# facebookresearch/dpr-scale

Hardware: NVIDIA H100
Metric: query+ctx pairs/sec (BERT-base, seq128) (higher is better)
Workload: dtype bf16

## Files before the change

dpr_scale_b200/csrc/attention.cu:

```cuda
#include "attention.cuh"
#include "dprb_internal.h"

namespace dprb {
namespace {

constexpr int DH = 64;
constexpr int SHORT_MAX = 256;

int check_shape(int nseq, int S, int heads, const char* who) {
  DPRB_REQUIRE(nseq >= 0 && heads > 0, "%s: bad nseq=%d heads=%d", who, nseq, heads);
  DPRB_REQUIRE(S >= 1 && S <= 512, "%s: sequence length %d unsupported (1..512)", who, S);
  return 0;
}

}

int attn_fwd_lse(const void* qkv, const int32_t* attn_mask, void* ctx, float* lse, int nseq, int S, int heads,
                 float dropout_p, unsigned long long site_seed, cudaStream_t stream) {
  if (int rc = check_shape(nseq, S, heads, "attn_fwd")) return rc;
  if (nseq == 0) return 0;
  if (S > SHORT_MAX) return attn_fwd_long(qkv, attn_mask, ctx, lse, nseq, S, heads, dropout_p, site_seed, stream);
  return attn_fwd_wg(qkv, attn_mask, ctx, lse, nseq, S, heads, dropout_p, site_seed, stream);
}

int attn_bwd_lse(const void* qkv, const int32_t* attn_mask, const void* ctx, const float* lse, const void* dctx,
                 void* dqkv, float* dbias, int nseq, int S, int heads, float dropout_p,
                 unsigned long long site_seed, cudaStream_t stream) {
  if (int rc = check_shape(nseq, S, heads, "attn_bwd")) return rc;
  if (nseq == 0) return 0;
  if (S > SHORT_MAX) {
    if (int rc = attn_bwd_long(qkv, attn_mask, ctx, lse, dctx, dqkv, nseq, S, heads, dropout_p, site_seed, stream)) return rc;
  } else {
    if (int rc = attn_bwd_wg(qkv, attn_mask, lse, dctx, dqkv, nseq, S, heads, dropout_p, site_seed, stream)) return rc;
  }
  if (dbias != nullptr) return colsum_bf16(dqkv, 3LL * heads * DH, dbias, nseq * S, 3 * heads * DH, stream);
  return 0;
}

}
```

dpr_scale_b200/csrc/attention_wgmma.cu:

```cuda
#include "attention.cuh"
#include "dprb_internal.h"

namespace dprb {
namespace {

template <int N>
__device__ __forceinline__ void mma_ss(float (&d)[N / 2], uint64_t a, uint64_t b, int acc) {
  if constexpr (N == 64) wgmma_m64n64_ss_bf16<0, 0>(d, a, b, acc);
  else if constexpr (N == 128) wgmma_m64n128_ss_bf16<0, 0>(d, a, b, acc);
  else wgmma_m64n256_ss_bf16<0, 0>(d, a, b, acc);
}

template <int NK>
constexpr int fwd_smem() { return 64 * 128 + 2 * NK * 128 + NK * 4 + 16 + 1024; }

template <int NK, bool DROP>
__global__ void __launch_bounds__(128)
attn_fwd_wg_kernel(const __grid_constant__ CUtensorMap tm_q, const __grid_constant__ CUtensorMap tm_kv,
                   const int32_t* __restrict__ attn_mask, bf16* __restrict__ ctx, float* __restrict__ lse_out, int S,
                   int heads, Drop drop) {
  extern __shared__ uint8_t smem_raw[];
  uint8_t* smem = align1024(smem_raw);
  uint8_t* sQ = smem;
  uint8_t* sK = sQ + 64 * 128;
  uint8_t* sV = sK + NK * 128;
  float* sMask = reinterpret_cast<float*>(sV + NK * 128);
  uint64_t* bar = reinterpret_cast<uint64_t*>(sMask + NK);

  const int tid = threadIdx.x, warp = tid >> 5, lane = tid & 31, q4 = lane & 3;
  const int nqb = (S + 63) / 64;
  const int prob = blockIdx.x / nqb, qb = blockIdx.x - prob * nqb;
  const int seq = prob / heads, h = prob - seq * heads;
  const int H = heads * 64;
  if (tid == 0) {
    tma_prefetch_desc(&tm_q);
    tma_prefetch_desc(&tm_kv);
    mbar_init(bar, 1);
    fence_barrier_init();
  }
  __syncthreads();
  if (tid == 0) {
    mbar_arrive_expect_tx(bar, 64 * 128 + 2 * NK * 128);
    tma_load_3d(sQ, &tm_q, bar, h * 64, qb * 64, seq);
    tma_load_3d(sK, &tm_kv, bar, H + h * 64, 0, seq);
    tma_load_3d(sV, &tm_kv, bar, 2 * H + h * 64, 0, seq);
  }
  for (int j = tid; j < NK; j += 128) {
    const bool keep = j < S && (attn_mask == nullptr || attn_mask[(long long)seq * S + j] != 0);
    sMask[j] = keep ? 0.f : -INFINITY;
  }
  __syncthreads();
  mbar_wait(bar, 0);

  float s[NK / 2];
  wgmma_fence();
#pragma unroll
  for (int k = 0; k < 4; ++k) mma_ss<NK>(s, desc_k(sQ) + k * KSTEP_K, desc_k(sK) + k * KSTEP_K, k > 0);
  wgmma_commit();
  wgmma_wait<0>();

  const int lrow = warp * 16 + (lane >> 2);
  float m[2] = {-INFINITY, -INFINITY};
#pragma unroll
  for (int c = 0; c < NK / 8; ++c) {
    const float2 mk = *reinterpret_cast<const float2*>(sMask + 8 * c + 2 * q4);
#pragma unroll
    for (int h2 = 0; h2 < 2; ++h2) {
      float& x = s[4 * c + 2 * h2];
      float& y = s[4 * c + 2 * h2 + 1];
      x = fmaf(x, ATTN_SCALE_LOG2, mk.x);
      y = fmaf(y, ATTN_SCALE_LOG2, mk.y);
      m[h2] = fmaxf(m[h2], fmaxf(x, y));
    }
  }
  float l[2] = {0.f, 0.f};
#pragma unroll
  for (int h2 = 0; h2 < 2; ++h2) {
    m[h2] = fmaxf(m[h2], __shfl_xor_sync(0xFFFFFFFFu, m[h2], 1));
    m[h2] = fmaxf(m[h2], __shfl_xor_sync(0xFFFFFFFFu, m[h2], 2));
  }
  const float e[2] = {m[0] == -INFINITY ? 0.f : m[0], m[1] == -INFINITY ? 0.f : m[1]};
  uint32_t pk[NK / 4];
#pragma unroll
  for (int c = 0; c < NK / 8; ++c) {
#pragma unroll
    for (int h2 = 0; h2 < 2; ++h2) {
      float px = ex2_approx(s[4 * c + 2 * h2] - e[h2]);
      float py = ex2_approx(s[4 * c + 2 * h2 + 1] - e[h2]);
      l[h2] += px + py;
      if (DROP) {
        float m0, m1;
        drop.mul2((uint32_t)(prob * S + qb * 64 + lrow + 8 * h2), (uint32_t)(8 * c + 2 * q4), m0, m1);
        px *= m0; py *= m1;
      }
      pk[2 * c + h2] = pack_bf16x2(px, py);
    }
  }
#pragma unroll
  for (int h2 = 0; h2 < 2; ++h2) {
    l[h2] += __shfl_xor_sync(0xFFFFFFFFu, l[h2], 1);
    l[h2] += __shfl_xor_sync(0xFFFFFFFFu, l[h2], 2);
  }

  float o[32];
  wgmma_fence();
#pragma unroll
  for (int j = 0; j < NK / 16; ++j) {
    const uint32_t a[4] = {pk[4 * j], pk[4 * j + 1], pk[4 * j + 2], pk[4 * j + 3]};
    wgmma_m64n64_rs_bf16<1>(o, a, desc_mn(sV) + j * KSTEP_MN, j > 0);
  }
  wgmma_commit();
  wgmma_wait<0>();

#pragma unroll
  for (int h2 = 0; h2 < 2; ++h2) {
    const int row = qb * 64 + lrow + 8 * h2;
    if (row >= S) continue;
    if (lse_out != nullptr && q4 == 0) lse_out[(long long)prob * S + row] = m[h2] * ATTN_LN2 + __logf(l[h2]);
    const float inv = l[h2] > 0.f ? 1.f / l[h2] : 0.f;
    bf16* dst = ctx + ((long long)seq * S + row) * H + h * 64;
#pragma unroll
    for (int c = 0; c < 8; ++c)
      *reinterpret_cast<uint32_t*>(dst + 8 * c + 2 * q4) = pack_bf16x2(o[4 * c + 2 * h2] * inv, o[4 * c + 2 * h2 + 1] * inv);
  }
}

template <int NK>
constexpr int bwd_smem() { return 4 * NK * 128 + NK * 256 + 2 * 8192 + 3 * NK * 4 + 16 + 1024; }

template <int NK, bool DROP>
__global__ void __launch_bounds__(256, 1)
attn_bwd_wg_kernel(const __grid_constant__ CUtensorMap tm_qkv, const __grid_constant__ CUtensorMap tm_do,
                   const int32_t* __restrict__ attn_mask, const float* __restrict__ lse_in, bf16* __restrict__ dqkv, int S,
                   int heads, Drop drop) {
  extern __shared__ uint8_t smem_raw[];
  uint8_t* smem = align1024(smem_raw);
  uint8_t* sQ = smem;
  uint8_t* sdO = sQ + NK * 128;
  uint8_t* sK = sdO + NK * 128;
  uint8_t* sV = sK + NK * 128;
  float* sdQ = reinterpret_cast<float*>(sV + NK * 128);
  uint8_t* sStage = reinterpret_cast<uint8_t*>(sdQ + NK * 64);
  float* sLse = reinterpret_cast<float*>(sStage + 2 * 8192);
  float* sD = sLse + NK;
  float* sMask = sD + NK;
  uint64_t* bar = reinterpret_cast<uint64_t*>(sMask + NK);

  const int tid = threadIdx.x, warp = tid >> 5, lane = tid & 31, q4 = lane & 3;
  const int wg = warp >> 2;
  const int prob = blockIdx.x, seq = prob / heads, h = prob - seq * heads;
  const int H = heads * 64;
  if (tid == 0) {
    tma_prefetch_desc(&tm_qkv);
    tma_prefetch_desc(&tm_do);
    mbar_init(bar, 1);
    fence_barrier_init();
  }
  __syncthreads();
  if (tid == 0) {
    mbar_arrive_expect_tx(bar, 4 * NK * 128);
    tma_load_3d(sQ, &tm_qkv, bar, h * 64, 0, seq);
    tma_load_3d(sdO, &tm_do, bar, h * 64, 0, seq);
    tma_load_3d(sK, &tm_qkv, bar, H + h * 64, 0, seq);
    tma_load_3d(sV, &tm_qkv, bar, 2 * H + h * 64, 0, seq);
  }
  for (int i = tid; i < NK * 64; i += 256) sdQ[i] = 0.f;
  for (int j = tid; j < NK; j += 256) {
    const bool keep = j < S && (attn_mask == nullptr || attn_mask[(long long)seq * S + j] != 0);
    sMask[j] = keep ? 0.f : -INFINITY;
    sLse[j] = j < S ? lse_in[(long long)prob * S + j] * ATTN_LOG2E : INFINITY;
    sD[j] = 0.f;
  }
  __syncthreads();
  mbar_wait(bar, 0);

  const int nblk = (S + 63) / 64;
  const int lrow = (warp & 3) * 16 + (lane >> 2);
  for (int qb = wg; qb < nblk; qb += 2) {
    float Dr[2] = {0.f, 0.f};
    const float ls[2] = {sLse[qb * 64 + lrow], sLse[qb * 64 + lrow + 8]};
    for (int kc = 0; kc < nblk; ++kc) {
      float sc[32], dp[32];
      wgmma_fence();
#pragma unroll
      for (int k = 0; k < 4; ++k) wgmma_m64n64_ss_bf16<0, 0>(sc, desc_k(sQ + qb * 8192) + k * KSTEP_K, desc_k(sK + kc * 8192) + k * KSTEP_K, k > 0);
#pragma unroll
      for (int k = 0; k < 4; ++k) wgmma_m64n64_ss_bf16<0, 0>(dp, desc_k(sdO + qb * 8192) + k * KSTEP_K, desc_k(sV + kc * 8192) + k * KSTEP_K, k > 0);
      wgmma_commit();
      wgmma_wait<0>();
#pragma unroll
      for (int c = 0; c < 8; ++c) {
        const int kcol = kc * 64 + 8 * c + 2 * q4;
        const float2 mk = *reinterpret_cast<const float2*>(sMask + kcol);
#pragma unroll
        for (int h2 = 0; h2 < 2; ++h2) {
          const int i = 4 * c + 2 * h2;
          float px = ex2_approx(fmaf(sc[i], ATTN_SCALE_LOG2, mk.x) - ls[h2]);
          float py = ex2_approx(fmaf(sc[i + 1], ATTN_SCALE_LOG2, mk.y) - ls[h2]);
          if (DROP) {
            float m0, m1;
            drop.mul2((uint32_t)(prob * S + qb * 64 + lrow + 8 * h2), (uint32_t)kcol, m0, m1);
            px *= m0; py *= m1;
          }
          Dr[h2] = fmaf(px, dp[i], fmaf(py, dp[i + 1], Dr[h2]));
        }
      }
    }
#pragma unroll
    for (int h2 = 0; h2 < 2; ++h2) {
      Dr[h2] += __shfl_xor_sync(0xFFFFFFFFu, Dr[h2], 1);
      Dr[h2] += __shfl_xor_sync(0xFFFFFFFFu, Dr[h2], 2);
      if (q4 == 0) sD[qb * 64 + lrow + 8 * h2] = Dr[h2];
    }
  }
  __syncthreads();

  uint8_t* stage = sStage + wg * 8192;
  for (int kb = wg; kb < nblk; kb += 2) {
    float dv[32], dk[32];
    const uint64_t dK_kb = desc_k(sK + kb * 64 * 128), dV_kb = desc_k(sV + kb * 64 * 128);
    const float mk[2] = {sMask[kb * 64 + lrow], sMask[kb * 64 + lrow + 8]};
    for (int qb = 0; qb < nblk; ++qb) {
      float st[32], dpt[32];
      wgmma_fence();
#pragma unroll
      for (int k = 0; k < 4; ++k) wgmma_m64n64_ss_bf16<0, 0>(st, dK_kb + k * KSTEP_K, desc_k(sQ + qb * 8192) + k * KSTEP_K, k > 0);
#pragma unroll
      for (int k = 0; k < 4; ++k) wgmma_m64n64_ss_bf16<0, 0>(dpt, dV_kb + k * KSTEP_K, desc_k(sdO + qb * 8192) + k * KSTEP_K, k > 0);
      wgmma_commit();
      wgmma_wait<0>();
      uint32_t pd[16], ds[16];
#pragma unroll
      for (int c = 0; c < 8; ++c) {
        const int qc = qb * 64 + 8 * c + 2 * q4;
        const float2 ls = *reinterpret_cast<const float2*>(sLse + qc);
        const float2 Dq = *reinterpret_cast<const float2*>(sD + qc);
#pragma unroll
        for (int h2 = 0; h2 < 2; ++h2) {
          const int i = 4 * c + 2 * h2;
          const float px = ex2_approx(fmaf(st[i], ATTN_SCALE_LOG2, mk[h2]) - ls.x);
          const float py = ex2_approx(fmaf(st[i + 1], ATTN_SCALE_LOG2, mk[h2]) - ls.y);
          float mx = 1.f, my = 1.f;
          if (DROP) {
            const uint32_t kr = (uint32_t)(kb * 64 + lrow + 8 * h2);
            mx = drop_one(drop, (uint32_t)(prob * S + qc), kr);
            my = drop_one(drop, (uint32_t)(prob * S + qc + 1), kr);
          }
          pd[2 * c + h2] = pack_bf16x2(px * mx, py * my);
          ds[2 * c + h2] = pack_bf16x2(px * fmaf(dpt[i], mx, -Dq.x) * 0.125f, py * fmaf(dpt[i + 1], my, -Dq.y) * 0.125f);
        }
      }
      named_bar_sync(1 + wg, 128);
#pragma unroll
      for (int c = 0; c < 8; ++c) {
#pragma unroll
        for (int h2 = 0; h2 < 2; ++h2) {
          const int r = lrow + 8 * h2;
          *reinterpret_cast<uint32_t*>(stage + r * 128 + ((c ^ (r & 7)) << 4) + q4 * 4) = ds[2 * c + h2];
        }
      }
      fence_proxy_async_smem();
      named_bar_sync(1 + wg, 128);
      float dq[32];
      wgmma_fence();
#pragma unroll
      for (int j = 0; j < 4; ++j) {
        const uint32_t a[4] = {pd[4 * j], pd[4 * j + 1], pd[4 * j + 2], pd[4 * j + 3]};
        wgmma_m64n64_rs_bf16<1>(dv, a, desc_mn(sdO + qb * 8192) + j * KSTEP_MN, qb > 0 || j > 0);
      }
#pragma unroll
      for (int j = 0; j < 4; ++j) {
        const uint32_t a[4] = {ds[4 * j], ds[4 * j + 1], ds[4 * j + 2], ds[4 * j + 3]};
        wgmma_m64n64_rs_bf16<1>(dk, a, desc_mn(sQ + qb * 8192) + j * KSTEP_MN, qb > 0 || j > 0);
      }
#pragma unroll
      for (int j = 0; j < 4; ++j)
        wgmma_m64n64_ss_bf16<1, 1>(dq, desc_mn(stage) + j * KSTEP_MN, desc_mn(sK + kb * 8192) + j * KSTEP_MN, j > 0);
      wgmma_commit();
      wgmma_wait<0>();
#pragma unroll
      for (int c = 0; c < 8; ++c) {
#pragma unroll
        for (int h2 = 0; h2 < 2; ++h2) {
          float* dst = sdQ + (qb * 64 + lrow + 8 * h2) * 64 + 8 * c + 2 * q4;
          atomicAdd(dst, dq[4 * c + 2 * h2]);
          atomicAdd(dst + 1, dq[4 * c + 2 * h2 + 1]);
        }
      }
    }
#pragma unroll
    for (int h2 = 0; h2 < 2; ++h2) {
      const int row = kb * 64 + lrow + 8 * h2;
      if (row >= S) continue;
      bf16* base = dqkv + ((long long)seq * S + row) * 3 * H + h * 64 + 2 * q4;
#pragma unroll
      for (int c = 0; c < 8; ++c) {
        *reinterpret_cast<uint32_t*>(base + H + 8 * c) = pack_bf16x2(dk[4 * c + 2 * h2], dk[4 * c + 2 * h2 + 1]);
        *reinterpret_cast<uint32_t*>(base + 2 * H + 8 * c) = pack_bf16x2(dv[4 * c + 2 * h2], dv[4 * c + 2 * h2 + 1]);
      }
    }
  }
  __syncthreads();
  for (int i = tid; i < S * 32; i += 256) {
    const int r = i >> 5, c2 = (i & 31) * 2;
    *reinterpret_cast<uint32_t*>(dqkv + ((long long)seq * S + r) * 3 * H + h * 64 + c2) =
        pack_bf16x2(sdQ[r * 64 + c2], sdQ[r * 64 + c2 + 1]);
  }
}

}

int make_tmap3(CUtensorMap* out, const void* base, int nseq, int S, long long cols, int box_rows) {
  DPRB_REQUIRE((reinterpret_cast<uintptr_t>(base) & 15) == 0 && cols % 8 == 0, "attention operand misaligned");
  const cuuint64_t dims[3] = {(cuuint64_t)cols, (cuuint64_t)S, (cuuint64_t)nseq};
  const cuuint64_t strides[2] = {(cuuint64_t)cols * 2, (cuuint64_t)S * cols * 2};
  const cuuint32_t box[3] = {64u, (cuuint32_t)box_rows, 1u};
  return encode_tmap(out, "attention", CU_TENSOR_MAP_DATA_TYPE_BFLOAT16, 3, base, dims, strides, box,
                     CU_TENSOR_MAP_L2_PROMOTION_L2_128B);
}

namespace {

template <int NK>
int fwd_launch(const CUtensorMap& tq, const CUtensorMap& tkv, const int32_t* attn_mask, void* ctx, float* lse, int nseq,
               int S, int heads, const Drop& drop, cudaStream_t stream) {
  constexpr int smem = fwd_smem<NK>();
  static bool attr = false;
  if (!attr) {
    DPRB_CHECK_CUDA(cudaFuncSetAttribute(attn_fwd_wg_kernel<NK, false>, cudaFuncAttributeMaxDynamicSharedMemorySize, smem));
    DPRB_CHECK_CUDA(cudaFuncSetAttribute(attn_fwd_wg_kernel<NK, true>, cudaFuncAttributeMaxDynamicSharedMemorySize, smem));
    attr = true;
  }
  const long long grid = (long long)((S + 63) / 64) * nseq * heads;
  DPRB_REQUIRE(grid < (1LL << 31), "attn_fwd: grid too large");
  if (drop.on()) attn_fwd_wg_kernel<NK, true><<<(unsigned)grid, 128, smem, stream>>>(tq, tkv, attn_mask, (bf16*)ctx, lse, S, heads, drop);
  else attn_fwd_wg_kernel<NK, false><<<(unsigned)grid, 128, smem, stream>>>(tq, tkv, attn_mask, (bf16*)ctx, lse, S, heads, drop);
  DPRB_LAUNCH_CHECK();
  return 0;
}

template <int NK>
int bwd_launch(const CUtensorMap& tq, const CUtensorMap& tdo, const int32_t* attn_mask, const float* lse, void* dqkv,
               int nseq, int S, int heads, const Drop& drop, cudaStream_t stream) {
  constexpr int smem = bwd_smem<NK>();
  static_assert(smem <= 227 * 1024, "attention backward: shared memory budget exceeded");
  static bool attr = false;
  if (!attr) {
    DPRB_CHECK_CUDA(cudaFuncSetAttribute(attn_bwd_wg_kernel<NK, false>, cudaFuncAttributeMaxDynamicSharedMemorySize, smem));
    DPRB_CHECK_CUDA(cudaFuncSetAttribute(attn_bwd_wg_kernel<NK, true>, cudaFuncAttributeMaxDynamicSharedMemorySize, smem));
    attr = true;
  }
  const int grid = nseq * heads;
  if (drop.on())
    attn_bwd_wg_kernel<NK, true><<<grid, 256, smem, stream>>>(tq, tdo, attn_mask, lse, (bf16*)dqkv, S, heads, drop);
  else
    attn_bwd_wg_kernel<NK, false><<<grid, 256, smem, stream>>>(tq, tdo, attn_mask, lse, (bf16*)dqkv, S, heads, drop);
  DPRB_LAUNCH_CHECK();
  return 0;
}

int pad_keys(int S) { return S <= 64 ? 64 : (S <= 128 ? 128 : 256); }

}

int attn_fwd_wg(const void* qkv, const int32_t* attn_mask, void* ctx, float* lse, int nseq, int S, int heads,
                float dropout_p, unsigned long long site_seed, cudaStream_t stream) {
  const Drop drop = drop_from_site(dropout_p, site_seed);
  const int H = heads * 64, NK = pad_keys(S);
  CUtensorMap tq, tkv;
  if (int rc = make_tmap3(&tq, qkv, nseq, S, 3LL * H, 64)) return rc;
  if (int rc = make_tmap3(&tkv, qkv, nseq, S, 3LL * H, NK)) return rc;
  if (NK == 64) return fwd_launch<64>(tq, tkv, attn_mask, ctx, lse, nseq, S, heads, drop, stream);
  if (NK == 128) return fwd_launch<128>(tq, tkv, attn_mask, ctx, lse, nseq, S, heads, drop, stream);
  return fwd_launch<256>(tq, tkv, attn_mask, ctx, lse, nseq, S, heads, drop, stream);
}

int attn_bwd_wg(const void* qkv, const int32_t* attn_mask, const float* lse, const void* dctx,
                void* dqkv, int nseq, int S, int heads, float dropout_p, unsigned long long site_seed,
                cudaStream_t stream) {
  const Drop drop = drop_from_site(dropout_p, site_seed);
  const int H = heads * 64, NK = pad_keys(S);
  DPRB_REQUIRE(lse != nullptr, "attn_bwd: lse from the forward is required");
  CUtensorMap tq, tdo;
  if (int rc = make_tmap3(&tq, qkv, nseq, S, 3LL * H, NK)) return rc;
  if (int rc = make_tmap3(&tdo, dctx, nseq, S, H, NK)) return rc;
  if (NK == 64) return bwd_launch<64>(tq, tdo, attn_mask, lse, dqkv, nseq, S, heads, drop, stream);
  if (NK == 128) return bwd_launch<128>(tq, tdo, attn_mask, lse, dqkv, nseq, S, heads, drop, stream);
  return bwd_launch<256>(tq, tdo, attn_mask, lse, dqkv, nseq, S, heads, drop, stream);
}

}
```

dpr_scale_b200/csrc/dprb_internal.h:

```cpp
#pragma once
#include <cuda.h>
#include <cuda_runtime.h>
#include "../../include/dprb.h"

namespace dprb {

int encode_tmap(CUtensorMap* out, const char* what, CUtensorMapDataType dtype, int rank, const void* base,
                const cuuint64_t* dims, const cuuint64_t* strides, const cuuint32_t* box,
                CUtensorMapL2promotion l2);

struct Carve {
  uint8_t* base;
  long long off;
  explicit Carve(void* b) : base(reinterpret_cast<uint8_t*>(b)), off(0) {}
  void* take(long long bytes) {
    void* p = base ? base + off : nullptr;
    off += (bytes + 255) & ~255LL;
    return p;
  }
};

int gemm_bf16(const void* A, const void* B, void* D, int M, int N, int K, long long lda, long long ldb,
              long long ldd, int a_mn_major, int b_mn_major, int epilogue, const float* bias, const void* aux,
              long long ld_aux, void* out2, float alpha, int splits, float* colsum, float dropout_p,
              unsigned long long drop_site_seed, cudaStream_t stream);

int gemm_profile_enable(int enable, int max_launches);
int gemm_profile_read(double* total_ms, double* total_flops, long long* launches);

int embed_ln_fwd(const int64_t* ids, const int64_t* type_ids, const int64_t* pos_ids, const float* word,
                 const float* pos, const float* type, const float* gamma, const float* beta, void* y, float* stats,
                 int T, int H, int vocab, int max_pos, int type_vocab, float eps, float dropout_p,
                 unsigned long long seed, void* y_res, cudaStream_t stream);
int embed_ln_bwd(const void* dy, const int64_t* ids, const int64_t* type_ids, const int64_t* pos_ids,
                 const float* word, const float* pos, const float* type, const float* gamma, const float* stats,
                 float* dword, float* dpos, float* dtype, float* dgamma, float* dbeta, int T, int H,
                 float dropout_p, unsigned long long seed, cudaStream_t stream);
int ln_fwd(const void* z, const float* gamma, const float* beta, void* y, float* stats, float* cls_out,
           int cls_stride, int T, int H, float eps, int z_f16, void* y_res, cudaStream_t stream);
int ln_bwd(const void* dy, const float* dy_cls, int cls_stride, const void* z, const float* stats,
           const float* gamma, void* dz, float* dgamma, float* dbeta, float* dbias, int T, int H, void* dzm,
           float dropout_p, unsigned long long site_seed, int z_f16, cudaStream_t stream);
int dropout_mask(uint8_t* out, long long rows, int cols, float p, unsigned long long seed, int layer, int site,
                 cudaStream_t stream);
unsigned long long drop_site_seed(unsigned long long seed, int layer, int site);
int gelu_from_pre(const void* pre, void* out, long long n, cudaStream_t stream);
int colsum_bf16(const void* x, long long ld, float* out, int T, int N, cudaStream_t stream);

int attn_fwd_lse(const void* qkv, const int32_t* attn_mask, void* ctx, float* lse, int nseq, int S, int heads,
                 float dropout_p, unsigned long long site_seed, cudaStream_t stream);
int attn_bwd_lse(const void* qkv, const int32_t* attn_mask, const void* ctx, const float* lse, const void* dctx,
                 void* dqkv, float* dbias, int nseq, int S, int heads, float dropout_p,
                 unsigned long long site_seed, cudaStream_t stream);

int attn_fwd_wg(const void* qkv, const int32_t* attn_mask, void* ctx, float* lse, int nseq, int S, int heads,
                float dropout_p, unsigned long long site_seed, cudaStream_t stream);
int attn_bwd_wg(const void* qkv, const int32_t* attn_mask, const float* lse, const void* dctx,
                void* dqkv, int nseq, int S, int heads, float dropout_p, unsigned long long site_seed,
                cudaStream_t stream);

int attn_cls_fwd(const void* qkv, const int32_t* attn_mask, void* ctx_cls, float* probs, int nseq, int S, int heads,
                 float dropout_p, unsigned long long site_seed, cudaStream_t stream);
int attn_cls_bwd(const void* qkv, const float* probs, const void* dctx_cls, void* dqkv, int nseq, int S, int heads,
                 float dropout_p, unsigned long long site_seed, cudaStream_t stream);
int add_rows_bf16(void* dst, const void* src, int nrows, int H, long long stride_rows, cudaStream_t stream);

int score_ce_fwd(const float* q, const float* c, const uint8_t* col_mask, const uint8_t* pair_mask,
                 const int64_t* labels, float inv_t, float* lse, float* loss_sum, float* logits, int Q, int C, int d,
                 cudaStream_t stream);
int score_ce_bwd(const float* q, const float* c, const float* logits, const int64_t* labels, const float* lse,
                 float grad_scale, float inv_t, float* dq, float* dc, int Q, int C, int d, int q0, int nq, int c0,
                 int nc, cudaStream_t stream);

bool score_tc_supported(int Q, int C, int d);
long long score_tc_workspace_bytes(int Q, int C, int d, int nq, int nc);
int score_tc_fwd(const float* q, const float* c, const uint8_t* col_mask, const uint8_t* pair_mask,
                 const int64_t* labels, float inv_t, float* lse, float* loss_sum, float* logits, int Q, int C, int d,
                 int nq, int nc, void* workspace, long long workspace_bytes, cudaStream_t stream);
int score_tc_bwd(const uint8_t* col_mask, const uint8_t* pair_mask, const int64_t* labels, const float* lse,
                 float grad_scale, float inv_t, float* dq, float* dc, int Q, int C, int d, int q0, int nq, int c0, int nc,
                 void* workspace, long long workspace_bytes, cudaStream_t stream);

int sumsq_f32(const float* g, long long n, float* out, cudaStream_t stream);
int adamw_step(float* p, const float* g, float* m, float* v, void* shadow, long long n, float lr, float beta1,
               float beta2, float eps, float wd, int step, float grad_scale, const float* sumsq, float max_norm,
               cudaStream_t stream);
int cast_f32_bf16(const float* src, void* dst, long long n, cudaStream_t stream);
int cast_bf16_f32(const void* src, float* dst, long long n, cudaStream_t stream);

long long search_workspace_bytes(long long Q, int k);
int search_topk(const void* queries, const void* corpus, int dtype, long long Q, long long N, int d, int k,
                long long index_offset, float* out_scores, long long* out_index, void* workspace,
                long long workspace_bytes, cudaStream_t stream);
long long topk_merge_workspace_bytes(long long Q, int total);
int topk_merge(const float* scores, const long long* index, long long Q, int total, int k, float* out_scores,
               long long* out_index, void* workspace, long long workspace_bytes, cudaStream_t stream);

int seqcls_head_fwd(const float* pre, const float* weight, const float* bias, float* logits, float* score, int N,
                    int H, int L, cudaStream_t stream);

long long encoder_workspace_bytes(const dprb_encoder_weights* w, int nseq, int S, int save);
int encoder_fwd(const dprb_encoder_weights* w, const dprb_encoder_batch* b, float* pooled, cudaStream_t stream);
int encoder_bwd(const dprb_encoder_weights* w, const dprb_encoder_batch* b, const float* dpooled, int layer_lo,
                int layer_hi, cudaStream_t stream);
int encoder_fwd_tokens(const dprb_encoder_weights* w, const dprb_encoder_batch* b, void* tokens, cudaStream_t stream);

int maxsim_fwd(const void* q, const void* d, const int32_t* q_mask, const int32_t* d_mask, const int32_t* q_index,
               int nq, int SQ, int B, int SD, int P, int pool, float* score, cudaStream_t stream);
int maxsim_expert_fwd(const void* q, const void* d, const int32_t* q_ids, const float* q_w, const int32_t* d_ids,
                      const float* d_w, const void* q_cls, const void* d_cls, const int32_t* q_index, int nq, int SQ,
                      int B, int SD, int P, int KQ, int KD, int Pc, int pool, float* score, cudaStream_t stream);

int splade_pool_fwd(const void* x, long long ldx, const void* W, long long ldw, const float* bias, const int32_t* off,
                    long long T, int N, int V, int K, float* out, long long ldo, cudaStream_t stream);

long long expert_group_workspace_bytes(int N, int S, int K);
int expert_group(const int32_t* ids, const float* w, const int32_t* mask, const int32_t* tokens, const void* reps,
                 long long ldr, int N, int S, int K, int P, int V, float threshold, int flags, int32_t* count,
                 int32_t* out_expert, int32_t* out_seq, int32_t* out_tok, float* out_w, float* out_payload,
                 void* workspace, long long workspace_bytes, cudaStream_t stream);

}
```

Measured before the change: 625.2.

## Add persistent short-sequence attention backward kernel with fused bias column sums

For sequences up to 128 tokens, attention backward now runs a new persistent kernel. Each CTA handles one head and loops over sequences, double-buffering the Q/dO/K/V tiles through TMA, and computes dQ, dK and dV with WGMMA in a single pass. The QKV bias gradient column sums are accumulated in shared memory and flushed with atomics, which removes the separate colsum pass over dqkv. The cost is a more complex kernel, float atomics whose summation order is not deterministic, and sizing the grid from occupancy queries.

```diff
diff --git a/dpr_scale_b200/csrc/attention.cu b/dpr_scale_b200/csrc/attention.cu
--- a/dpr_scale_b200/csrc/attention.cu
+++ b/dpr_scale_b200/csrc/attention.cu
@@ -28,11 +28,9 @@
                  unsigned long long site_seed, cudaStream_t stream) {
   if (int rc = check_shape(nseq, S, heads, "attn_bwd")) return rc;
   if (nseq == 0) return 0;
-  if (S > SHORT_MAX) {
-    if (int rc = attn_bwd_long(qkv, attn_mask, ctx, lse, dctx, dqkv, nseq, S, heads, dropout_p, site_seed, stream)) return rc;
-  } else {
-    if (int rc = attn_bwd_wg(qkv, attn_mask, lse, dctx, dqkv, nseq, S, heads, dropout_p, site_seed, stream)) return rc;
-  }
+  if (S <= SHORT_MAX)
+    return attn_bwd_wg(qkv, attn_mask, lse, dctx, dqkv, dbias, nseq, S, heads, dropout_p, site_seed, stream);
+  if (int rc = attn_bwd_long(qkv, attn_mask, ctx, lse, dctx, dqkv, nseq, S, heads, dropout_p, site_seed, stream)) return rc;
   if (dbias != nullptr) return colsum_bf16(dqkv, 3LL * heads * DH, dbias, nseq * S, 3 * heads * DH, stream);
   return 0;
 }
diff --git a/dpr_scale_b200/csrc/attention_wgmma.cu b/dpr_scale_b200/csrc/attention_wgmma.cu
--- a/dpr_scale_b200/csrc/attention_wgmma.cu
+++ b/dpr_scale_b200/csrc/attention_wgmma.cu
@@ -1,5 +1,7 @@
 #include "attention.cuh"
 #include "dprb_internal.h"
+
+#include <algorithm>
 
 namespace dprb {
 namespace {
@@ -122,6 +124,200 @@
 #pragma unroll
     for (int c = 0; c < 8; ++c)
       *reinterpret_cast<uint32_t*>(dst + 8 * c + 2 * q4) = pack_bf16x2(o[4 * c + 2 * h2] * inv, o[4 * c + 2 * h2 + 1] * inv);
+  }
+}
+
+__device__ __forceinline__ float2 rowlane_sum16(const float (&v)[16], int lane) {
+  const bool b2 = lane & 16, b1 = lane & 8, b0 = lane & 4;
+  float w[8], x[4], y[2];
+#pragma unroll
+  for (int j = 0; j < 8; ++j) w[j] = (b2 ? v[8 + j] : v[j]) + __shfl_xor_sync(0xFFFFFFFFu, b2 ? v[j] : v[8 + j], 16);
+#pragma unroll
+  for (int j = 0; j < 4; ++j) x[j] = (b1 ? w[4 + j] : w[j]) + __shfl_xor_sync(0xFFFFFFFFu, b1 ? w[j] : w[4 + j], 8);
+#pragma unroll
+  for (int j = 0; j < 2; ++j) y[j] = (b0 ? x[2 + j] : x[j]) + __shfl_xor_sync(0xFFFFFFFFu, b0 ? x[j] : x[2 + j], 4);
+  return make_float2(y[0], y[1]);
+}
+
+__device__ __forceinline__ void store_rows_colsum(const float (&acc)[32], bf16* dst, long long ld, int row0, int S,
+                                                  int q4, int lane, bool sums, float* sbias) {
+  float cs[16];
+#pragma unroll
+  for (int i = 0; i < 16; ++i) cs[i] = 0.f;
+#pragma unroll
+  for (int h2 = 0; h2 < 2; ++h2) {
+    const int row = row0 + 8 * h2;
+    if (row >= S) continue;
+#pragma unroll
+    for (int c = 0; c < 8; ++c) {
+      const uint32_t u = pack_bf16x2(acc[4 * c + 2 * h2], acc[4 * c + 2 * h2 + 1]);
+      *reinterpret_cast<uint32_t*>(dst + row * ld + 8 * c + 2 * q4) = u;
+      const float2 f = unpack_bf16x2(u);
+      cs[2 * c] += f.x;
+      cs[2 * c + 1] += f.y;
+    }
+  }
+  if (sums) {
+    const float2 t = rowlane_sum16(cs, lane);
+    float2* p = reinterpret_cast<float2*>(sbias + 8 * (lane >> 2) + 2 * q4);
+    *p = make_float2(p->x + t.x, p->y + t.y);
+  }
+}
+
+template <int NK>
+constexpr int bwd_short_smem() { return 8 * NK * 128 + 2 * NK * NK * 2 + 2 * NK * 4 + (NK / 16) * 192 * 4 + 16 + 1024; }
+
+template <int NK, bool DROP>
+__global__ void __launch_bounds__(2 * NK, NK == 64 ? 2 : 1)
+attn_bwd_short_kernel(const __grid_constant__ CUtensorMap tm_qkv, const __grid_constant__ CUtensorMap tm_do,
+                      const int32_t* __restrict__ attn_mask, const float* __restrict__ lse_in, bf16* __restrict__ dqkv,
+                      float* __restrict__ dbias, int nseq, int S, int heads, Drop drop) {
+  constexpr int NT = 2 * NK, NWARP = NT / 32, OPS = NK * 128, BUF = 4 * OPS, STG = NK * NK * 2;
+  extern __shared__ uint8_t smem_raw[];
+  uint8_t* smem = align1024(smem_raw);
+  uint8_t* sP = smem + 2 * BUF;
+  uint8_t* sdS = sP + STG;
+  float* sMask = reinterpret_cast<float*>(sdS + STG);
+  float* sBias = sMask + 2 * NK;
+  uint64_t* bar = reinterpret_cast<uint64_t*>(sBias + NWARP * 192);
+
+  const int tid = threadIdx.x, warp = tid >> 5, lane = tid & 31, q4 = lane & 3;
+  const int wg = warp >> 2;
+  const int lrow = (warp & 3) * 16 + (lane >> 2);
+  const int h = blockIdx.x % heads, stride = gridDim.x / heads;
+  const int H = heads * 64;
+  const bool sums = dbias != nullptr;
+
+  auto load = [&](int seq, int b) {
+    uint8_t* buf = smem + b * BUF;
+    mbar_arrive_expect_tx(&bar[b], BUF);
+    tma_load_3d(buf, &tm_qkv, &bar[b], h * 64, 0, seq);
+    tma_load_3d(buf + OPS, &tm_do, &bar[b], h * 64, 0, seq);
+    tma_load_3d(buf + 2 * OPS, &tm_qkv, &bar[b], H + h * 64, 0, seq);
+    tma_load_3d(buf + 3 * OPS, &tm_qkv, &bar[b], 2 * H + h * 64, 0, seq);
+  };
+  auto fill_mask = [&](int seq, int b) {
+    if (tid < NK) {
+      const bool keep = tid < S && (attn_mask == nullptr || attn_mask[(long long)seq * S + tid] != 0);
+      sMask[b * NK + tid] = keep ? 0.f : -INFINITY;
+    }
+  };
+
+  const int seq0 = blockIdx.x / heads;
+  if (tid == 0) {
+    tma_prefetch_desc(&tm_qkv);
+    tma_prefetch_desc(&tm_do);
+    mbar_init(&bar[0], 1);
+    mbar_init(&bar[1], 1);
+    fence_barrier_init();
+  }
+  for (int i = tid; i < NWARP * 192; i += NT) sBias[i] = 0.f;
+  if (seq0 < nseq) fill_mask(seq0, 0);
+  __syncthreads();
+  if (tid == 0 && seq0 < nseq) load(seq0, 0);
+
+  int it = 0;
+  for (int seq = seq0; seq < nseq; seq += stride, ++it) {
+    const int b = it & 1;
+    const int prob = seq * heads + h;
+    if (seq + stride < nseq) {
+      if (tid == 0) load(seq + stride, b ^ 1);
+      fill_mask(seq + stride, b ^ 1);
+    }
+    const uint8_t* sQ = smem + b * BUF;
+    const uint8_t* sdO = sQ + OPS;
+    const uint8_t* sK = sQ + 2 * OPS;
+    const uint8_t* sV = sQ + 3 * OPS;
+    const float* mask = sMask + b * NK;
+    const int r0 = wg * 64 + lrow;
+    float ls[2];
+#pragma unroll
+    for (int h2 = 0; h2 < 2; ++h2)
+      ls[h2] = r0 + 8 * h2 < S ? lse_in[(long long)prob * S + r0 + 8 * h2] * ATTN_LOG2E : INFINITY;
+    mbar_wait(&bar[b], (it >> 1) & 1);
+
+    float s[NK / 2], dp[NK / 2];
+    wgmma_fence();
+#pragma unroll
+    for (int k = 0; k < 4; ++k) mma_ss<NK>(s, desc_k(sQ + wg * 8192) + k * KSTEP_K, desc_k(sK) + k * KSTEP_K, k > 0);
+#pragma unroll
+    for (int k = 0; k < 4; ++k) mma_ss<NK>(dp, desc_k(sdO + wg * 8192) + k * KSTEP_K, desc_k(sV) + k * KSTEP_K, k > 0);
+    wgmma_commit();
+    wgmma_wait<0>();
+
+    float D[2] = {0.f, 0.f};
+#pragma unroll
+    for (int c = 0; c < NK / 8; ++c) {
+      const float2 mk = *reinterpret_cast<const float2*>(mask + 8 * c + 2 * q4);
+#pragma unroll
+      for (int h2 = 0; h2 < 2; ++h2) {
+        const int i = 4 * c + 2 * h2, r = r0 + 8 * h2;
+        const float px = ex2_approx(fmaf(s[i], ATTN_SCALE_LOG2, mk.x) - ls[h2]);
+        const float py = ex2_approx(fmaf(s[i + 1], ATTN_SCALE_LOG2, mk.y) - ls[h2]);
+        float m0 = 1.f, m1 = 1.f;
+        if (DROP) {
+          drop.mul2((uint32_t)(prob * S + r), (uint32_t)(8 * c + 2 * q4), m0, m1);
+          dp[i] *= m0;
+          dp[i + 1] *= m1;
+        }
+        s[i] = px;
+        s[i + 1] = py;
+        D[h2] = fmaf(px, dp[i], fmaf(py, dp[i + 1], D[h2]));
+        *reinterpret_cast<uint32_t*>(sP + (c >> 3) * (NK * 128) + r * 128 + (((c & 7) ^ (r & 7)) << 4) + q4 * 4) =
+            pack_bf16x2(px * m0, py * m1);
+      }
+    }
+#pragma unroll
+    for (int h2 = 0; h2 < 2; ++h2) {
+      D[h2] += __shfl_xor_sync(0xFFFFFFFFu, D[h2], 1);
+      D[h2] += __shfl_xor_sync(0xFFFFFFFFu, D[h2], 2);
+    }
+    uint32_t ds[NK / 4];
+#pragma unroll
+    for (int c = 0; c < NK / 8; ++c) {
+#pragma unroll
+      for (int h2 = 0; h2 < 2; ++h2) {
+        const int i = 4 * c + 2 * h2, r = r0 + 8 * h2;
+        ds[2 * c + h2] = pack_bf16x2(s[i] * (dp[i] - D[h2]) * 0.125f, s[i + 1] * (dp[i + 1] - D[h2]) * 0.125f);
+        *reinterpret_cast<uint32_t*>(sdS + (c >> 3) * (NK * 128) + r * 128 + (((c & 7) ^ (r & 7)) << 4) + q4 * 4) =
+            ds[2 * c + h2];
+      }
+    }
+    float dq[32];
+    wgmma_fence();
+#pragma unroll
+    for (int j = 0; j < NK / 16; ++j) {
+      const uint32_t a[4] = {ds[4 * j], ds[4 * j + 1], ds[4 * j + 2], ds[4 * j + 3]};
+      wgmma_m64n64_rs_bf16<1>(dq, a, desc_mn(sK) + j * KSTEP_MN, j > 0);
+    }
+    wgmma_commit();
+    fence_proxy_async_smem();
+    __syncthreads();
+
+    float dv[32], dk[32];
+    wgmma_fence();
+#pragma unroll
+    for (int j = 0; j < NK / 16; ++j)
+      wgmma_m64n64_ss_bf16<1, 1>(dv, desc_mn(sP + wg * (NK * 128)) + j * KSTEP_MN, desc_mn(sdO) + j * KSTEP_MN, j > 0);
+#pragma unroll
+    for (int j = 0; j < NK / 16; ++j)
+      wgmma_m64n64_ss_bf16<1, 1>(dk, desc_mn(sdS + wg * (NK * 128)) + j * KSTEP_MN, desc_mn(sQ) + j * KSTEP_MN, j > 0);
+    wgmma_commit();
+    bf16* out = dqkv + (long long)seq * S * 3 * H + h * 64;
+    wgmma_wait<1>();
+    store_rows_colsum(dq, out, 3LL * H, wg * 64 + lrow, S, q4, lane, sums, sBias + warp * 192);
+    wgmma_wait<0>();
+    store_rows_colsum(dk, out + H, 3LL * H, wg * 64 + lrow, S, q4, lane, sums, sBias + warp * 192 + 64);
+    store_rows_colsum(dv, out + 2 * H, 3LL * H, wg * 64 + lrow, S, q4, lane, sums, sBias + warp * 192 + 128);
+    __syncthreads();
+  }
+  if (sums && it > 0) {
+    for (int t = tid; t < 192; t += NT) {
+      float v = 0.f;
+#pragma unroll
+      for (int w = 0; w < NWARP; ++w) v += sBias[w * 192 + t];
+      atomicAdd(dbias + (t >> 6) * H + h * 64 + (t & 63), v);
+    }
   }
 }
 
@@ -339,22 +535,48 @@
   return 0;
 }
 
-template <int NK>
 int bwd_launch(const CUtensorMap& tq, const CUtensorMap& tdo, const int32_t* attn_mask, const float* lse, void* dqkv,
                int nseq, int S, int heads, const Drop& drop, cudaStream_t stream) {
-  constexpr int smem = bwd_smem<NK>();
+  constexpr int smem = bwd_smem<256>();
   static_assert(smem <= 227 * 1024, "attention backward: shared memory budget exceeded");
   static bool attr = false;
   if (!attr) {
-    DPRB_CHECK_CUDA(cudaFuncSetAttribute(attn_bwd_wg_kernel<NK, false>, cudaFuncAttributeMaxDynamicSharedMemorySize, smem));
-    DPRB_CHECK_CUDA(cudaFuncSetAttribute(attn_bwd_wg_kernel<NK, true>, cudaFuncAttributeMaxDynamicSharedMemorySize, smem));
+    DPRB_CHECK_CUDA(cudaFuncSetAttribute(attn_bwd_wg_kernel<256, false>, cudaFuncAttributeMaxDynamicSharedMemorySize, smem));
+    DPRB_CHECK_CUDA(cudaFuncSetAttribute(attn_bwd_wg_kernel<256, true>, cudaFuncAttributeMaxDynamicSharedMemorySize, smem));
     attr = true;
   }
   const int grid = nseq * heads;
   if (drop.on())
-    attn_bwd_wg_kernel<NK, true><<<grid, 256, smem, stream>>>(tq, tdo, attn_mask, lse, (bf16*)dqkv, S, heads, drop);
+    attn_bwd_wg_kernel<256, true><<<grid, 256, smem, stream>>>(tq, tdo, attn_mask, lse, (bf16*)dqkv, S, heads, drop);
   else
-    attn_bwd_wg_kernel<NK, false><<<grid, 256, smem, stream>>>(tq, tdo, attn_mask, lse, (bf16*)dqkv, S, heads, drop);
+    attn_bwd_wg_kernel<256, false><<<grid, 256, smem, stream>>>(tq, tdo, attn_mask, lse, (bf16*)dqkv, S, heads, drop);
+  DPRB_LAUNCH_CHECK();
+  return 0;
+}
+
+template <int NK>
+int bwd_short_launch(const CUtensorMap& tq, const CUtensorMap& tdo, const int32_t* attn_mask, const float* lse,
+                     void* dqkv, float* dbias, int nseq, int S, int heads, const Drop& drop, cudaStream_t stream) {
+  constexpr int smem = bwd_short_smem<NK>();
+  static_assert(smem <= 227 * 1024, "attention backward: shared memory budget exceeded");
+  static int per_sm = 0;
+  if (per_sm == 0) {
+    DPRB_CHECK_CUDA(cudaFuncSetAttribute(attn_bwd_short_kernel<NK, false>, cudaFuncAttributeMaxDynamicSharedMemorySize, smem));
+    DPRB_CHECK_CUDA(cudaFuncSetAttribute(attn_bwd_short_kernel<NK, true>, cudaFuncAttributeMaxDynamicSharedMemorySize, smem));
+    int n = 0;
+    DPRB_CHECK_CUDA(cudaOccupancyMaxActiveBlocksPerMultiprocessor(&n, attn_bwd_short_kernel<NK, true>, 2 * NK, smem));
+    DPRB_REQUIRE(n > 0, "attn_bwd: the S <= %d kernel does not fit on an SM", NK);
+    per_sm = n;
+  }
+  DPRB_NUM_SMS(sms);
+  const int per_head = std::max(1, std::min(nseq, per_sm * sms / heads));
+  const int grid = per_head * heads;
+  if (drop.on())
+    attn_bwd_short_kernel<NK, true><<<grid, 2 * NK, smem, stream>>>(tq, tdo, attn_mask, lse, (bf16*)dqkv, dbias, nseq,
+                                                                    S, heads, drop);
+  else
+    attn_bwd_short_kernel<NK, false><<<grid, 2 * NK, smem, stream>>>(tq, tdo, attn_mask, lse, (bf16*)dqkv, dbias, nseq,
+                                                                     S, heads, drop);
   DPRB_LAUNCH_CHECK();
   return 0;
 }
@@ -376,7 +598,7 @@
 }
 
 int attn_bwd_wg(const void* qkv, const int32_t* attn_mask, const float* lse, const void* dctx,
-                void* dqkv, int nseq, int S, int heads, float dropout_p, unsigned long long site_seed,
+                void* dqkv, float* dbias, int nseq, int S, int heads, float dropout_p, unsigned long long site_seed,
                 cudaStream_t stream) {
   const Drop drop = drop_from_site(dropout_p, site_seed);
   const int H = heads * 64, NK = pad_keys(S);
@@ -384,9 +606,10 @@
   CUtensorMap tq, tdo;
   if (int rc = make_tmap3(&tq, qkv, nseq, S, 3LL * H, NK)) return rc;
   if (int rc = make_tmap3(&tdo, dctx, nseq, S, H, NK)) return rc;
-  if (NK == 64) return bwd_launch<64>(tq, tdo, attn_mask, lse, dqkv, nseq, S, heads, drop, stream);
-  if (NK == 128) return bwd_launch<128>(tq, tdo, attn_mask, lse, dqkv, nseq, S, heads, drop, stream);
-  return bwd_launch<256>(tq, tdo, attn_mask, lse, dqkv, nseq, S, heads, drop, stream);
-}
-
-}
+  if (NK == 64) return bwd_short_launch<64>(tq, tdo, attn_mask, lse, dqkv, dbias, nseq, S, heads, drop, stream);
+  if (NK == 128) return bwd_short_launch<128>(tq, tdo, attn_mask, lse, dqkv, dbias, nseq, S, heads, drop, stream);
+  if (int rc = bwd_launch(tq, tdo, attn_mask, lse, dqkv, nseq, S, heads, drop, stream)) return rc;
+  return dbias != nullptr ? colsum_bf16(dqkv, 3LL * H, dbias, nseq * S, 3 * H, stream) : 0;
+}
+
+}
diff --git a/dpr_scale_b200/csrc/dprb_internal.h b/dpr_scale_b200/csrc/dprb_internal.h
--- a/dpr_scale_b200/csrc/dprb_internal.h
+++ b/dpr_scale_b200/csrc/dprb_internal.h
@@ -56,7 +56,7 @@
 int attn_fwd_wg(const void* qkv, const int32_t* attn_mask, void* ctx, float* lse, int nseq, int S, int heads,
                 float dropout_p, unsigned long long site_seed, cudaStream_t stream);
 int attn_bwd_wg(const void* qkv, const int32_t* attn_mask, const float* lse, const void* dctx,
-                void* dqkv, int nseq, int S, int heads, float dropout_p, unsigned long long site_seed,
+                void* dqkv, float* dbias, int nseq, int S, int heads, float dropout_p, unsigned long long site_seed,
                 cudaStream_t stream);
 
 int attn_cls_fwd(const void* qkv, const int32_t* attn_mask, void* ctx_cls, float* probs, int nseq, int S, int heads,
```

Result: faster. 754.4 (median of 6 runs) (+20.7%).
